# jdeschut/tunempc

Measured on AMD Instinct MI355X. Metric: stage-Hessian convexifications/sec at (nx+nu)=32, p=64, higher is better.
Workload: dtype f64

## Files before the change

### include/tunempc_hip.h

```cpp
#ifndef TUNEMPC_HIP_H
#define TUNEMPC_HIP_H

#include <stdint.h>

#ifdef __cplusplus
extern "C" {
#endif

#define TMPC_OK 0
#define TMPC_E_ARG (-1)
#define TMPC_E_UNSUPPORTED (-2)
#define TMPC_E_NOMEM (-3)
#define TMPC_E_HIP (-4)
#define TMPC_E_NODEVICE (-5)
#define TMPC_E_NOCONV (-6)

#define TMPC_STATUS_OPTIMAL 0
#define TMPC_STATUS_FEASIBLE 1
#define TMPC_STATUS_INFEASIBLE 2

#define TMPC_FLAG_NO_MFMA 1
#define TMPC_FLAG_PROFILE 2
#define TMPC_FLAG_FAST_EXIT 4

// ... 14 lines not shown
int tmpc_create_con(tmpc_handle** out, int chunk, int p, int nx, int mb, int ng, int nc);
int tmpc_destroy(tmpc_handle* h);
int tmpc_get_chunk(tmpc_handle* h);

int tmpc_set_options(tmpc_handle* h, double tol, double center_tol, int max_iter, int center_iter, int flags);

#define TMPC_TUNE_CHORD_STEP 1
#define TMPC_TUNE_SMALL_BLOCKS 2
#define TMPC_TUNE_EIG_PRETEST 3
#define TMPC_TUNE_FUSE_FWD 4
#define TMPC_TUNE_GRAPH 5
#define TMPC_TUNE_PERSISTENT 7
#define TMPC_TUNE_LOWP_SWITCH 8
#define TMPC_LOWP_SWITCH_DEFAULT 1e-5
#define TMPC_TUNE_LOWP_TRSM 9
int tmpc_set_tuning(tmpc_handle* h, int key, double value);
int tmpc_create_ex(tmpc_handle** out, int chunk, int p, int nx, int mb, int ng, int nc, int step3, int lanes);

int tmpc_set_tight(tmpc_handle* h, int enable, double tight_tol);

int tmpc_convexify_batch_host(tmpc_handle* h, int nb, const double* A, const double* B, const double* H,
                              double* Hc, double* dHc, double* P, double* alpha, double* beta, double* kappa,
                              int32_t* status, int32_t* iters, double* info);
int tmpc_convexify_batch_device(tmpc_handle* h, int nb, const double* dA, const double* dB, const double* dH,
                                double* dHc_out, double* ddHc_out, double* dP_out, double* d_alpha, double* d_beta,
                                double* d_kappa, int32_t* d_status, int32_t* d_iters, double* d_info, void* stream);

int tmpc_convexify_eq_batch_host(tmpc_handle* h, int nb, const double* A, const double* B, const double* H, const double* G,
                                 double* Hc, double* dHc, double* P, double* Fg, double* alpha, double* beta, double* kappa,
                                 int32_t* status, int32_t* iters, double* info);
// ... 77 lines not shown
```

### include/tunempc_hip_debug.h

```cpp
#ifndef TUNEMPC_HIP_DEBUG_H
#define TUNEMPC_HIP_DEBUG_H

#include "tunempc_hip.h"

#ifdef __cplusplus
extern "C" {
#endif

#define TMPC_DEBUG_FLAG_STOP_ASSEMBLED 8
#define TMPC_DEBUG_FLAG_NO_LIFT 16
#define TMPC_DEBUG_FLAG_NO_DMA 32
#define TMPC_DEBUG_FLAG_GENERIC_STAGE 64

int tmpc_debug_gemm_nt(tmpc_handle* h, double* C, const double* A, const double* B, int M, int N, int K, int mode, int lower);

int tmpc_debug_block_solve(tmpc_handle* h, int p, int d, const double* D, const double* Ccpl, const double* rhs, double* x, int32_t* nshift);

#define TMPC_DEBUG_FACTOR_PASS1 1
#define TMPC_DEBUG_FACTOR_FUSE_FWD1 2
#define TMPC_DEBUG_FACTOR_LOWP_TRSM 4
#define TMPC_DEBUG_FACTOR_DD 8
typedef struct {
  const double *D, *Ccpl, *Dlo, *Clo, *rhs;
  const int32_t *list, *lowp;
  double *oD, *oO, *oF, *oDdiag, *oX;
  float* oO32;
  double *oDl, *oOl, *oFl, *oXl;
  int32_t *nshift, *dims, *orient;
} tmpc_debug_factor_io;
int tmpc_debug_block_factor(tmpc_handle* h, int nb, int p, int d, int count, int mode, const tmpc_debug_factor_io* io);

int tmpc_debug_cr_schedule(int p, int32_t* out, int cap);

int tmpc_debug_get_multipliers(tmpc_handle* h, int nb, int nr, double* phi, double* z, double* dphi, double* dz);

int tmpc_debug_get_array(tmpc_handle* h, int which, uint64_t offset, uint64_t count, double* out);

int tmpc_debug_min_eig(tmpc_handle* h, int nmat, int n, const double* W, double* out);
int tmpc_debug_min_eig_lane(tmpc_handle* h, int nmat, int n, const double* W, double* out);

int tmpc_debug_factor_bench(tmpc_handle* h, int nb, int p, int d, int reps, double* ms_out2);

#ifdef __cplusplus
// ... 4 lines not shown
```

### tunempc_amd/_lib.py

```python
import ctypes as C
import os

import numpy as np

_HERE = os.path.dirname(os.path.abspath(__file__))
_LIB = None

INFO_STRIDE = 16
FLAG_NO_MFMA = 1
FLAG_PROFILE = 2
FLAG_FAST_EXIT = 4
STATUS_NAMES = {0: 'Optimal', 1: 'Feasible', 2: 'Infeasible'}

ARROW_LD = 32
EXPORTS = [
    'tmpc_device_count', 'tmpc_workspace_bytes', 'tmpc_workspace_bytes_eq', 'tmpc_workspace_bytes_con',
    'tmpc_create', 'tmpc_create_eq', 'tmpc_create_con', 'tmpc_destroy', 'tmpc_get_chunk', 'tmpc_set_options', 'tmpc_set_tight', 'tmpc_set_tuning', 'tmpc_create_ex',
    'tmpc_convexify_batch_host', 'tmpc_convexify_batch_device', 'tmpc_convexify_eq_batch_host', 'tmpc_convexify_step2_batch_host',
    'tmpc_convexify_con_batch_device', 'tmpc_workspace_bytes_step3', 'tmpc_create_step3', 'tmpc_convexify_step3_batch_host', 'tmpc_workspace_bytes_step3_con', 'tmpc_create_step3_con', 'tmpc_convexify_step3_con_batch_host', 'tmpc_convexify_step3_batch_device', 'tmpc_convexify_step3_con_batch_device', 'tmpc_supplement_batch_host', 'tmpc_supplement_terms_batch_host',
    'tmpc_tracking_reference_host', 'tmpc_eig_scan_host', 'tmpc_get_profile', 'tmpc_get_trace', 'tmpc_get_dual_host', 'tmpc_get_dual_con_host', 'tmpc_pack_sensitivities_host', 'tmpc_eig_clip_host',
    'tmpc_periodic_lqr_batch_host', 'tmpc_periodic_lqr_batch_device', 'tmpc_periodic_lqr_rows_batch_host', 'tmpc_periodic_lqr_rows_batch_device',
    'tmpc_periodic_lqr_ctg_batch_host', 'tmpc_periodic_lqr_ctg_batch_device',
    'tmpc_last_error', 'tmpc_version',
]
DEBUG_EXPORTS = [
    'tmpc_debug_gemm_nt', 'tmpc_debug_block_solve', 'tmpc_debug_cr_schedule', 'tmpc_debug_get_multipliers', 'tmpc_debug_get_array',
    'tmpc_debug_min_eig', 'tmpc_debug_min_eig_lane', 'tmpc_debug_factor_bench', 'tmpc_debug_block_factor',
]
FLAG_DEBUG_NO_DMA = 32
FACTOR_PASS1, FACTOR_FUSE_FWD1, FACTOR_LOWP_TRSM, FACTOR_DD = 1, 2, 4, 8


class _FactorIO(C.Structure):
    _fields_ = ([(n, C.POINTER(C.c_double)) for n in ('D', 'Ccpl', 'Dlo', 'Clo', 'rhs')] + [(n, C.POINTER(C.c_int32)) for n in ('list', 'lowp')] +
                [(n, C.POINTER(C.c_double)) for n in ('oD', 'oO', 'oF', 'oDdiag', 'oX')] + [('oO32', C.POINTER(C.c_float))] +
                [(n, C.POINTER(C.c_double)) for n in ('oDl', 'oOl', 'oFl', 'oXl')] + [(n, C.POINTER(C.c_int32)) for n in ('nshift', 'dims', 'orient')])


def library_path():
    return os.environ.get('TMPC_LIB') or os.path.join(_HERE, 'lib', 'libtunempc_hip.so')


def load_library():
    global _LIB
    if _LIB is not None:
        return _LIB
    path = library_path()
    if not os.path.exists(path):
        raise RuntimeError(
            f"tunempc_amd: HIP library not built ({path}); run `python -c 'import __graft_entry__ as g; g.build()'`"
            " -- there is no CPU fallback for the convexify hot path")
# ... 148 lines not shown
            _check(self.lib, self.lib.tmpc_create_step3_con(C.byref(self._h), int(chunk), self.p, self.nx, self.mb, self.ng, self.nc), 'tmpc_create_step3_con')
        elif self.step3:
            _check(self.lib, self.lib.tmpc_create_step3(C.byref(self._h), int(chunk), self.p, self.nx, self.mb), 'tmpc_create_step3')
        else:
            _check(self.lib, self.lib.tmpc_create_con(C.byref(self._h), int(chunk), self.p, self.nx, self.mb, self.ng, self.nc), 'tmpc_create_con')
        self.chunk = int(self.lib.tmpc_get_chunk(self._h))
        self.flags = int(flags)
        self.set_options(tol, center_tol, max_iter, center_iter, flags)

    def set_options(self, tol=None, center_tol=None, max_iter=None, center_iter=None, flags=None):
        if flags is not None:
            self.flags = int(flags)
        _check(self.lib, self.lib.tmpc_set_options(self._h, float(tol or 0.0), float(center_tol or 0.0),
                                                   int(max_iter or 0), int(center_iter or 0), self.flags), 'tmpc_set_options')

    def set_tuning(self, chord_step=None, small_blocks=None, eig_pretest=None, fuse_fwd=None, graph=None, persistent=None, lowp_switch=None, lowp_trsm=None):
        for key, v in ((1, chord_step), (2, small_blocks), (3, eig_pretest), (4, fuse_fwd), (5, graph), (7, persistent), (8, lowp_switch), (9, lowp_trsm)):
            if v is not None:
                _check(self.lib, self.lib.tmpc_set_tuning(self._h, key, float(v)), 'tmpc_set_tuning')

    def set_tight(self, enable=True, tight_tol=None):
        _check(self.lib, self.lib.tmpc_set_tight(self._h, 1 if enable else 0, float(tight_tol or 0.0)), 'tmpc_set_tight')

    def close(self):
        if getattr(self, '_h', None) is not None and self._h.value:
            self.lib.tmpc_destroy(self._h)
            self._h = C.c_void_p()

    def __del__(self):
        try:
            self.close()
        except Exception:
# ... 305 lines not shown
        nc = 3 if pass1 else 1
        if Ccpl.shape != D.shape or rhs.shape != ((nb, p, d, 3) if pass1 else (nb, p, d)):
            raise ValueError('debug_block_factor: D, Ccpl [nb, p, d, d] and rhs [nb, p, d] (pass 2) / [nb, p, d, 3] (pass 1) expected')
        plist = np.ascontiguousarray(np.arange(nb) if plist is None else plist, dtype=np.int32)
        lowp = None if lowp is None else np.ascontiguousarray(lowp, dtype=np.int32)
        if lowp is not None and lowp.shape != (nb,):
            raise ValueError('debug_block_factor: lowp [nb] expected')
        mode = (FACTOR_PASS1 if pass1 else 0) | (FACTOR_FUSE_FWD1 if fuse_fwd1 else 0) | (FACTOR_LOWP_TRSM if lowp_trsm else 0) | (FACTOR_DD if dd else 0)
        dp = (d + 15) // 16 * 16; ld32 = (dp + 31) // 32 * 32
        has32 = bool(lowp_trsm or (lowp is not None and lowp.any()))
        raw = dict(D=np.empty((nb, p, dp, dp)), O=np.empty((nb, p, dp, dp)), F=np.empty((nb, p, dp, dp)), Ddiag=np.empty((nb, p, dp)), X=np.empty((nb, p, dp, nc)),
                   O32=np.empty((nb, 2 * p, dp, ld32), np.float32) if has32 else None)
        if dd:
            raw.update(Dl=np.empty((nb, p, dp, dp)), Ol=np.empty((nb, p, dp, dp)), Fl=np.empty((nb, p, dp, dp)), Xl=np.empty((nb, p, dp, nc)))
        nshift = np.zeros(nb, np.int32); dims = np.zeros(4, np.int32); orient = np.zeros(p, np.int32)
        io = _FactorIO(D=_dptr(D), Ccpl=_dptr(Ccpl), Dlo=_dptr(Dlo), Clo=_dptr(Clo), rhs=_dptr(rhs), list=_iptr(plist), lowp=_iptr(lowp),
                       oD=_dptr(raw['D']), oO=_dptr(raw['O']), oF=_dptr(raw['F']), oDdiag=_dptr(raw['Ddiag']), oX=_dptr(raw['X']),
                       oO32=raw['O32'].ctypes.data_as(C.POINTER(C.c_float)) if has32 else None,
                       oDl=_dptr(raw.get('Dl')), oOl=_dptr(raw.get('Ol')), oFl=_dptr(raw.get('Fl')), oXl=_dptr(raw.get('Xl')),
                       nshift=_iptr(nshift), dims=_iptr(dims), orient=_iptr(orient))
        _check(self.lib, self.lib.tmpc_debug_block_factor(self._h, nb, p, d, len(plist), mode, C.byref(io)), 'tmpc_debug_block_factor')
        assert (int(dims[0]), int(dims[1]), int(dims[2]), bool(dims[3])) == (dp, ld32, nc, has32), dims
        raw.update(dp=dp, ld32=ld32)
        cut = lambda a: None if a is None else a[:, :, :d, :d].copy()
        vec = lambda a: None if a is None else (a[:, :, :d, :].copy() if pass1 else a[:, :, :d, 0].copy())
        out = dict(raw=raw, orient=orient, nshift=nshift, D=cut(raw['D']), L=np.tril(cut(raw['D'])), O=cut(raw['O']), F=cut(raw['F']), O32=cut(raw['O32']),
                   Ddiag=raw['Ddiag'][:, :, :d].copy(), x=vec(raw['X']))
        if dd:
            out.update(Dl=cut(raw['Dl']), Ll=np.tril(cut(raw['Dl'])), Ol=cut(raw['Ol']), Fl=cut(raw['Fl']), xl=vec(raw['Xl']))
        return out


def eig_clip(A, tol):
    lib = load_library()
    A = np.ascontiguousarray(A, dtype=np.float64)
    single = A.ndim == 2
    A3 = A[None] if single else A
    nb, n, n2 = A3.shape
    if n != n2:
        raise ValueError('square matrices expected')
    out = np.empty_like(A3); ev = np.empty((nb, n)); reg = np.empty(nb); sw = np.zeros(nb, dtype=np.int32)
    rc = lib.tmpc_eig_clip_host(nb, n, _dptr(A3), float(tol), _dptr(out), _dptr(ev), _dptr(reg), _iptr(sw))
# ... 124 lines not shown
```

### tunempc_amd/csrc/tmpc_api.hip

```cpp
#include <hip/hip_runtime.h>
#include <stdio.h>
#include <stdlib.h>
#include <new>
#include <string.h>
#include <algorithm>
#include <chrono>
#include <thread>
#include <mutex>
#include <condition_variable>
#include <functional>
#include <unistd.h>
#include <vector>

#include <string>
#include <unordered_map>

#include "../../include/tunempc_hip.h"
#include "../../include/tunempc_hip_debug.h"
#include "tmpc_common.h"
#include "tmpc_small.h"
#include "tmpc_stage.h"
#include "tmpc_schur.h"
#include "tmpc_factor.h"
#include "tmpc_cr.h"
// ... 92 lines not shown

struct tmpc_handle {
  Dims dm;
  int chunk;
  int nlanes;
  Opts opt;
  int flags;
  Lane lane[MAXL];
  void* slab;
  size_t slab_bytes;
  hipEvent_t ev_in;
  int device;
  CrSched sched;
  int* d_sched;
  int rs, mt;
  int tune_small, tune_pretest, tune_fuse, tune_graph, tune_persist, tune_lowp_trsm;
  void* dd_slab;
  size_t dd_bytes;
  int tight;
  double tight_tol;
};

static int cr_upload(const CrSched& sc, int** out) {
  std::vector<int> flat(sc.elim);
  flat.insert(flat.end(), sc.upd.begin(), sc.upd.end());
  flat.insert(flat.end(), sc.orient.begin(), sc.orient.end());
  *out = nullptr;
  if (hipMalloc(out, flat.size() * sizeof(int)) != hipSuccess) return TMPC_E_NOMEM;
  if (hipMemcpy(*out, flat.data(), flat.size() * sizeof(int), hipMemcpyHostToDevice) != hipSuccess) { hipFree(*out); *out = nullptr; return TMPC_E_HIP; }
  return TMPC_OK;
}
// ... 498 lines not shown
  } while (0)

static int run_chunk(tmpc_handle* h, Lane* ln, int nb, const double* dA, const double* dB, const double* dH, hipStream_t st,
                     const double* dG = nullptr, const int32_t* dncnt = nullptr, double rho = 0.0, bool step3 = false) {
  Dims dm = h->dm;
  dm.B = nb;
  if (!step3) dm.nT = 0;
  if (!dG) { dm.ng = 0; dm.nr = 0; dm.nz = 0; }
  dm.constr = (dG && dncnt && rho > 0.0) ? 1 : 0;
  if (dG && !dncnt) { dm.nr = dm.ng; dm.nz = dm.ng; }
  if (dG && dncnt && !dm.constr) dm.nz = dm.nr;
  const bool eq = dm.nr > 0;
  const bool t3 = dm.nT > 0;
  dm.dp = (dm.d + (eq ? dm.nz : 0) + (t3 ? dm.nT + 1 : 0) + 15) / 16 * 16;
  dm.nt = (dm.dp + TB - 1) / TB;
  dm.flags = (h->flags & TMPC_FLAG_NO_MFMA) | (h->tune_small ? 0 : DF_NO_SMALL) | ((h->flags & TMPC_DEBUG_FLAG_NO_DMA) ? DF_NO_DMA : 0);
  const size_t t3_lds = (size_t)(3 * (dm.nT + 1) + 8) * sizeof(double);
  const bool big = dm.n > NMAX || (h->flags & TMPC_DEBUG_FLAG_GENERIC_STAGE);
  const size_t t3_schur_lds = (size_t)((big ? 0 : 9 * 32 * T3_LD) + 2 * (dm.nT + 1)) * sizeof(double) + (size_t)(2 * (dm.nT + 1) + 2 * (dm.d + 1)) * sizeof(short) + 64;
  if (big && !ln->ws.bscr) {
    if (hipMalloc(&ln->big_scr, (size_t)h->dm.B * dm.p * BIG_SCR * dm.n * dm.n * sizeof(double)) != hipSuccess) { snprintf(g_err, sizeof(g_err), "hipMalloc of the generic-stage scratch failed"); return TMPC_E_NOMEM; }
    ln->ws.bscr = (double*)ln->big_scr;
  }
  WS wall = ln->ws;
  wall.A = dA; wall.Bm = dB; wall.H = dH; wall.G = dG; wall.ncnt = dncnt; wall.rho = rho;
  wall.cr_orient = h->d_sched + h->sched.elim.size() + h->sched.upd.size();
  WS w = wall;
  w.A = nullptr; w.Bm = nullptr; w.H = nullptr;
  int* alist = wall.alist;
  int* flist = wall.flist;
  wall.alist = nullptr;
// ... 348 lines not shown
  }
  tmpc_handle* h = new (std::nothrow) tmpc_handle();
  if (!h) return TMPC_E_NOMEM;
  h->slab = nullptr; h->d_sched = nullptr; h->ev_in = nullptr; h->dd_slab = nullptr; h->dd_bytes = 0; h->tight = 0; h->tight_tol = 0x1p-37;
  if (hipGetDevice(&h->device) != hipSuccess) { delete h; return TMPC_E_HIP; }
  int nl = (make_dims(1, p, nx, mb, ng, nc, step3).dp <= 64 && chunk >= 2) ? 2 : 1;
  if (lanes >= 1) nl = std::min(lanes, MAXL);
  nl = std::max(1, std::min(nl, chunk));
  h->nlanes = nl;
  const int cap = (chunk + nl - 1) / nl;
  h->chunk = cap * nl;
  h->dm = make_dims(cap, p, nx, mb, ng, nc, step3);
  h->sched = cr_build(p);
  h->rs = 0; h->mt = 0;
  h->tune_small = 1; h->tune_pretest = 1; h->tune_fuse = 1; h->tune_graph = 1; h->tune_persist = 1; h->tune_lowp_trsm = 1;
  h->opt.tol = 0x1p-25; h->opt.center_tol = 1e-9; h->opt.max_iter = 50; h->opt.center_iter = 12;
  h->opt.fast_exit = 0;
  h->opt.lowp_switch = TMPC_LOWP_SWITCH_DEFAULT;
  h->opt.chord_step = 10.0;
  h->flags = 0;
  WS tmp;
  const size_t lane_bytes = carve(tmp, h->dm, nullptr, nullptr);
  h->slab_bytes = lane_bytes * nl;
  if (hipMalloc(&h->slab, h->slab_bytes) != hipSuccess) {
    snprintf(g_err, sizeof(g_err), "hipMalloc(%zu bytes) failed", h->slab_bytes);
    delete h;
    return TMPC_E_NOMEM;
  }
  int rc = cr_upload(h->sched, &h->d_sched);
  bool ok = (rc == TMPC_OK) && hipEventCreateWithFlags(&h->ev_in, hipEventDisableTiming) == hipSuccess;
// ... 51 lines not shown
  return TMPC_OK;
}


int tmpc_set_tuning(tmpc_handle* h, int key, double value) {
  if (!h) return TMPC_E_ARG;
  switch (key) {
    case TMPC_TUNE_CHORD_STEP: if (!(value >= 0.0)) return TMPC_E_ARG; h->opt.chord_step = value; return TMPC_OK;
    case TMPC_TUNE_LOWP_SWITCH: if (!(value >= 0.0)) return TMPC_E_ARG; h->opt.lowp_switch = value; return TMPC_OK;
    case TMPC_TUNE_SMALL_BLOCKS: h->tune_small = value != 0.0; return TMPC_OK;
    case TMPC_TUNE_EIG_PRETEST: h->tune_pretest = value != 0.0; return TMPC_OK;
    case TMPC_TUNE_FUSE_FWD: h->tune_fuse = value != 0.0; return TMPC_OK;
    case TMPC_TUNE_GRAPH: h->tune_graph = value != 0.0; return TMPC_OK;
    case TMPC_TUNE_PERSISTENT: if (!(value >= 0.0 && value <= 2.0)) return TMPC_E_ARG; h->tune_persist = (int)value; return TMPC_OK;
    case TMPC_TUNE_LOWP_TRSM: h->tune_lowp_trsm = value != 0.0; return TMPC_OK;
    default: snprintf(g_err, sizeof(g_err), "tmpc_set_tuning: unknown key %d", key); return TMPC_E_ARG;
  }
}

int tmpc_set_tight(tmpc_handle* h, int enable, double tight_tol) {
  if (!h) return TMPC_E_ARG;
  if (!enable) { h->tight = 0; return TMPC_OK; }
  if (h->dm.nT > 0) { snprintf(g_err, sizeof(g_err), "tmpc_set_tight: Steps 1 and 2 only (no Step 3 handles)"); return TMPC_E_UNSUPPORTED; }
  if (h->dm.nr > 0 && (size_t)dd_aug_lds_doubles(h->dm.nr, h->dm.n, h->dm.nx) * sizeof(double) > 160 * 1024) {
    snprintf(g_err, sizeof(g_err), "tmpc_set_tight: %d rows per stage at nx = %d, nx + mb = %d: their double-double vectors do not fit the LDS (rows * (2 n + 2 nx) <= 4040)", h->dm.nr, h->dm.nx, h->dm.n);
    return TMPC_E_UNSUPPORTED;
  }
  if ((size_t)dd_solve_lds_doubles(h->dm.dp) * sizeof(double) > 160 * 1024) {
    snprintf(g_err, sizeof(g_err), "tmpc_set_tight: Schur blocks of %d do not fit the LDS image of the double-double substitution kernels (nx <= 51)", h->dm.dp);
    return TMPC_E_UNSUPPORTED;
// ... 810 lines not shown
        double dv = (i == j) ? 1.0 : 0.0, cv = 0.0;
        if (i < d && j < d) { dv = D[((size_t)k * d + i) * d + j]; cv = Ccpl[((size_t)k * d + i) * d + j]; }
        hD[k * bs + (size_t)i * dp + j] = dv;
        if (sc.orient[k]) hO[k * bs + (size_t)i * dp + j] = cv; else hO[k * bs + (size_t)j * dp + i] = cv;
      }
    for (int i = 0; i < d; ++i) hdd[(size_t)k * dp + i] = D[((size_t)k * d + i) * d + i];
  }
}

int tmpc_debug_block_solve(tmpc_handle* h, int p, int d, const double* D, const double* Ccpl, const double* rhs, double* x, int32_t* nshift) {
  if (!h || p < 1 || d < 1 || !D || !Ccpl || !rhs || !x) return TMPC_E_ARG;
  ON_DEVICE(h);
  CrBench cb;
  int rc = cb.init(1, p, d, h->flags, h->opt.lowp_switch >= 1.0);
  if (rc != TMPC_OK) return rc;
  const int dp = cb.dm.dp;
  const size_t bs = (size_t)dp * dp;
  std::vector<double> hD, hO, hdd, hz((size_t)p * dp, 0.0);
  cr_pack(cb.sc, p, d, dp, D, Ccpl, hD, hO, hdd);
  for (int k = 0; k < p; ++k) for (int i = 0; i < d; ++i) hz[(size_t)k * dp + i] = rhs[(size_t)k * d + i];
  HIPCHK(hipMemcpy(cb.w.D, hD.data(), p * bs * 8, hipMemcpyHostToDevice));
  HIPCHK(hipMemcpy(cb.w.O, hO.data(), p * bs * 8, hipMemcpyHostToDevice));
  HIPCHK(hipMemcpy(cb.w.Ddiag, hdd.data(), (size_t)p * dp * 8, hipMemcpyHostToDevice));
  HIPCHK(hipMemcpy(cb.w.Z, hz.data(), (size_t)p * dp * 8, hipMemcpyHostToDevice));
  cr_factor(cb.w, cb.dm, cb.sc, cb.d_sched, cb.w.alist, 1, 0, h->rs, h->mt, nullptr, nullptr, 0, cb.w.O32 ? 1 : 0);
  cr_solve(cb.w, cb.dm, cb.sc, cb.d_sched, cb.w.alist, 1, 0, 2);
  HIPCHK(hipDeviceSynchronize());
  HIPCHK(hipGetLastError());
  int hip_[IS];
  HIPCHK(hipMemcpy(hz.data(), cb.w.Z, (size_t)p * dp * 8, hipMemcpyDeviceToHost));
// ... 8 lines not shown
  if (mode & ~(TMPC_DEBUG_FACTOR_PASS1 | TMPC_DEBUG_FACTOR_FUSE_FWD1 | TMPC_DEBUG_FACTOR_LOWP_TRSM | TMPC_DEBUG_FACTOR_DD)) return TMPC_E_ARG;
  const bool pass1 = (mode & TMPC_DEBUG_FACTOR_PASS1) != 0, fuse = (mode & TMPC_DEBUG_FACTOR_FUSE_FWD1) != 0, ddm = (mode & TMPC_DEBUG_FACTOR_DD) != 0;
  std::vector<char> seen(nb, 0);
  int nlowp = 0, anylowp = 0;
  for (int i = 0; i < count; ++i) {
    const int b = io->list[i];
    if (b < 0 || b >= nb || seen[b]) { snprintf(g_err, sizeof(g_err), "tmpc_debug_block_factor: list entry %d is out of range or repeated", i); return TMPC_E_ARG; }
    seen[b] = 1;
    if (io->lowp && io->lowp[b]) ++nlowp;
  }
  for (int b = 0; b < nb && io->lowp; ++b) anylowp |= io->lowp[b] != 0;
  ON_DEVICE(h);
  CrBench cb;
  int rc = cb.init(nb, p, d, h->flags, false);
  if (rc != TMPC_OK) return rc;
  Dims& dm = cb.dm; WS& w = cb.w;
  if (h->flags & TMPC_DEBUG_FLAG_NO_DMA) dm.flags |= DF_NO_DMA;
  if (!h->tune_small) dm.flags |= DF_NO_SMALL;
  const int dp = dm.dp, ld32 = (dp + 31) & ~31, nc = pass1 ? 3 : 1;
  const size_t bs = (size_t)dp * dp, per = (size_t)p * bs, vl = (size_t)p * dp;
  if (solve_lds(dm) > 160 * 1024) return TMPC_E_UNSUPPORTED;
  const bool lowp_ok = !(dm.flags & (1 | DF_NO_DMA)) && dp > 64 && dm.nt <= TRR_NT;
  const bool fuse_ok = pass1 && !(dm.flags & (1 | DF_NO_DMA)) && p > 1 && dm.nt <= TRR_NT && !cr_small_levels(dm, cb.sc, nullptr);
  if ((anylowp || (mode & TMPC_DEBUG_FACTOR_LOWP_TRSM)) && (!lowp_ok || ddm)) { snprintf(g_err, sizeof(g_err), "tmpc_debug_block_factor: no float32 path at dp = %d with these flags", dp); return TMPC_E_ARG; }
  if (fuse && (!fuse_ok || ddm)) { snprintf(g_err, sizeof(g_err), "tmpc_debug_block_factor: no fused forward sweep at p = %d, dp = %d with these flags", p, dp); return TMPC_E_ARG; }
  DevBuf O32b, Dlb, Olb, Flb, Lilb, W3lb, Zlb;
  const size_t n32 = 2 * (size_t)nb * p * dp * ld32;
  if (anylowp || (mode & TMPC_DEBUG_FACTOR_LOWP_TRSM)) {
    if (O32b.alloc(n32 * sizeof(float)) != hipSuccess) return TMPC_E_NOMEM;
    HIPCHK(hipMemset(O32b.p, 0, n32 * sizeof(float)));
// ... 20 lines not shown
      std::fill(hz.begin(), hz.end(), 0.0);
      for (int k = 0; k < p; ++k) for (int i = 0; i < d; ++i) for (int q = 0; q < nc; ++q) hz[((size_t)k * dp + i) * nc + q] = io->rhs[(((size_t)b * p + k) * d + i) * nc + q];
      HIPCHK(hipMemcpy(w.D + b * per, hD.data(), per * 8, hipMemcpyHostToDevice));
      HIPCHK(hipMemcpy(w.O + b * per, hO.data(), per * 8, hipMemcpyHostToDevice));
      HIPCHK(hipMemcpy(w.Ddiag + b * vl, hdd.data(), vl * 8, hipMemcpyHostToDevice));
      HIPCHK(hipMemcpy(X + b * vl * nc, hz.data(), vl * nc * 8, hipMemcpyHostToDevice));
      if (ddm) {
        cr_pack(cb.sc, p, d, dp, io->Dlo ? io->Dlo + b * dd_ : zero.data(), io->Clo ? io->Clo + b * dd_ : zero.data(), hDl, hOl, hdl);
        for (int k = 0; k < p; ++k) for (int i = d; i < dp; ++i) hDl[k * bs + (size_t)i * dp + i] = 0.0;
        HIPCHK(hipMemcpy(w.Dl + b * per, hDl.data(), per * 8, hipMemcpyHostToDevice));
        HIPCHK(hipMemcpy(w.Ol + b * per, hOl.data(), per * 8, hipMemcpyHostToDevice));
      }
    }
  }
  if (count > 0) HIPCHK(hipMemcpy(w.alist, io->list, (size_t)count * sizeof(int), hipMemcpyHostToDevice));
  if (anylowp) {
    std::vector<int> hi((size_t)nb * IS, 0);
    for (int b = 0; b < nb; ++b) hi[(size_t)b * IS + I_LOWP] = io->lowp[b] ? 1 : 0;
    HIPCHK(hipMemcpy(w.iprob, hi.data(), hi.size() * sizeof(int), hipMemcpyHostToDevice));
  }
  if (count > 0) {
    const int pass = pass1 ? 1 : 2;
    if (ddm) {
      dd_factor(w, dm, cb.sc, cb.d_sched, w.alist, count, 0);
      rc = dd_solve(w, dm, cb.sc, cb.d_sched, w.alist, count, 0, pass, nb);
      if (rc != TMPC_OK) return rc;
    } else {
      cr_factor(w, dm, cb.sc, cb.d_sched, w.alist, count, 0, h->rs, h->mt, nullptr, nullptr, fuse ? 1 : 0, nlowp);
      cr_solve(w, dm, cb.sc, cb.d_sched, w.alist, count, 0, pass, fuse);
    }
// ... 7 lines not shown
  if (io->oX) HIPCHK(hipMemcpy(io->oX, X, nb * vl * nc * 8, hipMemcpyDeviceToHost));
  if (io->oO32 && w.O32) HIPCHK(hipMemcpy(io->oO32, w.O32, n32 * sizeof(float), hipMemcpyDeviceToHost));
  if (ddm) {
    if (io->oDl) HIPCHK(hipMemcpy(io->oDl, w.Dl, nb * per * 8, hipMemcpyDeviceToHost));
    if (io->oOl) HIPCHK(hipMemcpy(io->oOl, w.Ol, nb * per * 8, hipMemcpyDeviceToHost));
    if (io->oFl) HIPCHK(hipMemcpy(io->oFl, w.Fl, nb * per * 8, hipMemcpyDeviceToHost));
    if (io->oXl) HIPCHK(hipMemcpy(io->oXl, Xl, nb * vl * nc * 8, hipMemcpyDeviceToHost));
  }
  if (io->nshift) {
    std::vector<int> hi((size_t)nb * IS);
    HIPCHK(hipMemcpy(hi.data(), w.iprob, hi.size() * sizeof(int), hipMemcpyDeviceToHost));
    for (int b = 0; b < nb; ++b) io->nshift[b] = hi[(size_t)b * IS + I_NSHIFT];
  }
  if (io->dims) { io->dims[0] = dp; io->dims[1] = ld32; io->dims[2] = nc; io->dims[3] = w.O32 ? 1 : 0; }
  if (io->orient) for (int k = 0; k < p; ++k) io->orient[k] = cb.sc.orient[k];
  return TMPC_OK;
}

int tmpc_debug_factor_bench(tmpc_handle* h, int nb, int p, int d, int reps, double* ms_out2) {
  if (!h || nb < 1 || p < 1 || d < 1 || reps < 1 || !ms_out2) return TMPC_E_ARG;
  ON_DEVICE(h);
  CrBench cb;
  cb.ablate = (int)h->opt.lowp_switch - 2;
  int rc = cb.init(nb, p, d, h->flags, h->opt.lowp_switch >= 1.0);
  if (rc != TMPC_OK) return rc;
  const int dp = cb.dm.dp;
  const size_t bs = (size_t)dp * dp, per = (size_t)p * bs;
  std::vector<double> E((size_t)p * d * d), G((size_t)p * d * d), Dd((size_t)p * d * d, 0.0), Cc((size_t)p * d * d, 0.0);
  unsigned long long st = 88172645463325252ull;
  auto rnd = [&]() { st ^= st << 13; st ^= st >> 7; st ^= st << 17; return ((double)(st % 2000001) / 1000000.0 - 1.0) / sqrt((double)d); };
  for (auto& v : E) v = rnd();
  for (auto& v : G) v = rnd();
  for (int k = 0; k < p; ++k) {
    const int kn = (k + 1) % p;
    const double* Ek = &E[(size_t)k * d * d]; const double* Gk = &G[(size_t)k * d * d];
    for (int i = 0; i < d; ++i)
      for (int j = 0; j < d; ++j) {
        double ee = 0, gg = 0, eg = 0;
        for (int r = 0; r < d; ++r) { ee += Ek[r * d + i] * Ek[r * d + j]; gg += Gk[r * d + i] * Gk[r * d + j]; eg += Ek[r * d + i] * Gk[r * d + j]; }
        Dd[((size_t)k * d + i) * d + j] += ee + (i == j ? 1.0 : 0.0); Dd[((size_t)kn * d + i) * d + j] += gg;
// ... 47 lines not shown
```

### tunempc_amd/csrc/tmpc_common.h

```cpp
#pragma once
#include <hip/hip_runtime.h>
#include <stdint.h>

namespace tmpc {

#ifdef TMPC_CYCLE_PROF
__device__ unsigned long long g_prof[64];
__device__ int g_prof_cls;
#define TMPC_T(i) { if (blockIdx.x == 0 && threadIdx.x == 0) { const unsigned long long t_ = __builtin_readcyclecounter(); g_prof[(g_prof_cls & 7) * 8 + (i)] += t_ - tprev_; tprev_ = t_; } }
#define TMPC_T0() unsigned long long tprev_ = __builtin_readcyclecounter();
#define TMPC_TC(c, i) { if (blockIdx.x == 0 && threadIdx.x == 0) { const unsigned long long t_ = __builtin_readcyclecounter(); g_prof[(c) * 8 + (i)] += t_ - tprevc_; tprevc_ = t_; } }
#define TMPC_TC0() unsigned long long tprevc_ = __builtin_readcyclecounter();
#else
#define TMPC_TC(c, i)
#define TMPC_TC0()
#define TMPC_T(i)
#define TMPC_T0()
#endif



constexpr double ALPHA_MIN = 1e-8;
constexpr int TRACE_LEN = 80, TRACE_W = 10;
constexpr int TB = 64;
// ... 36 lines not shown
  int p;
  int nx, mb;
  int n;
  int d;
  int dp;
  int nt;
  int flags;
  int ng;
  int nr;
  int nz;
  int constr;
  int nT;
};
constexpr int DF_LOWP = 8;
constexpr int DF_LOWP_TRSM = 16;
constexpr int NGM = 31;
constexpr int NCM = 31;
constexpr int NRM = NGM + NCM, NZM = NRM + 2;
constexpr int NRS = 32, NZS = NRS + 2;
constexpr int NAM = 31;
constexpr int AEL = NAM + 1, AE = AEL * AEL;

struct Opts {
  double tol;
  double center_tol;
  int max_iter;
  int center_iter;
  double chord_step;
  int tight;
  double tight_tol;
// ... 80 lines not shown
```

### tunempc_amd/csrc/tmpc_cr.h

```cpp
#pragma once
#include <climits>
#include <vector>

#include "tmpc_common.h"
#include "tmpc_factor.h"
#include "tmpc_gemm_dma.h"

namespace tmpc {

constexpr int CR_EW = 8;
constexpr int CR_UW = 8;
enum { CE_NODE = 0, CE_NA, CE_NB, CE_EA, CE_EB, CE_FILL, CE_FX, CE_FACC };
enum { CU_NODE = 0, CU_E0, CU_S0, CU_E1, CU_S1 };

struct CrLevel { int eoff, nelim, uoff, nupd; };
struct CrSched {
  int p = 0;
  int prep = 0;
  std::vector<int> orient;
  std::vector<int> elim, upd;
  std::vector<CrLevel> lev;
};

static inline CrSched cr_build(int p) {
// ... 130 lines not shown

constexpr int UPD_DMA_DEPTH = 2;
template <bool USE_MFMA>
__global__ void __launch_bounds__(256, 2) k_cr_potrf(WS w, Dims dm, CrDev cr, int eoff, int nelim, int count) {
  const int it = cr_item(count * nelim);
  if (it < 0) return;
  extern __shared__ __attribute__((aligned(16))) double lds[];
  const int b = cr.alist[it / nelim];
  const int* er = cr.elim + (size_t)(eoff + it % nelim) * CR_EW;
  const int node = er[CE_NODE], dp = dm.dp;
  const size_t bs = (size_t)dp * dp;
  double* Dk = w.D + ((size_t)b * dm.p + node) * bs;
  double* Li = w.Linv + ((size_t)b * dm.p + node) * dm.nt * TB * TB;
  const double* dref = w.Ddiag + ((size_t)b * dm.p + node) * dp;
  double minr = 1.0;
  const int nbad = wg_block_column<USE_MFMA>(Dk, nullptr, nullptr, Li, dref, dp, lds, &minr);
  if (threadIdx.x == 0) {
    if (nbad) atomicAdd(w.iprob + (size_t)b * IS + I_NSHIFT, nbad);
    if (w.prob && minr < 1.0) atomic_min_pos(w.prob + (size_t)b * PS + P_MINPIV, minr);
  }
}

template <bool USE_MFMA, int NS>
__global__ void __launch_bounds__(256, 2) k_cr_trsm(WS w, Dims dm, CrDev cr, int eoff, int nelim, int count, int rs) {
  const int nstrip = (dm.dp + rs - 1) / rs;
  const int per = 2 * nstrip;
  const int it = cr_item(count * nelim * per);
  if (it < 0) return;
  extern __shared__ __attribute__((aligned(16))) double lds[];
  const int g = it / per, r = it - g * per;
  const int b = cr.alist[g / nelim];
// ... 586 lines not shown
  extern __shared__ __attribute__((aligned(16))) double lds[];
  const int b = cr.alist[it / nelim];
  const int* er = cr.elim + (size_t)(eoff + it % nelim) * CR_EW;
  const int node = er[CE_NODE], dp = dm.dp;
  double* Dk = w.D + ((size_t)b * dm.p + node) * (size_t)dp * dp;
  double* Li = w.Linv + ((size_t)b * dm.p + node) * dm.nt * TB * TB;
  const double* dref = w.Ddiag + ((size_t)b * dm.p + node) * dp;
  double* stat = lds + FACT_LDS_DOUBLES - 8;
  if (threadIdx.x == 0) { stat[0] = 0.0; stat[1] = 1.0; }
  for (int r = 0; r < dm.nt; ++r) {
    const int r0 = 64 * r, nb = (dp - r0 < 64) ? dp - r0 : 64;
    if (r > 0) {
      trd_strip<true>(Dk + (size_t)r0 * dp, Dk, Li, nb, r + 1, dp, it, lds);
      __syncthreads();
    }
    wg_potrf_inv(Dk + (size_t)r0 * dp + r0, dp, Li + (size_t)r * TB * TB, dref + r0, nb, lds, nullptr, stat, (it >> 5) & 3, r > 0);
  }
  if (threadIdx.x == 0) {
    const int nbad = (int)stat[0];
    const double minr = stat[1];
    if (nbad) atomicAdd(w.iprob + (size_t)b * IS + I_NSHIFT, nbad);
    if (w.prob && minr < 1.0) atomic_min_pos(w.prob + (size_t)b * PS + P_MINPIV, minr);
  }
}

template <bool USE_MFMA, int NS>
__global__ void __launch_bounds__(256, 2) k_cr_update(WS w, Dims dm, CrDev cr, int eoff, int nelim, int uoff, int nupd, int count, int mt) {
  const int nm = (dm.dp + mt - 1) / mt;
  const int ntl = nm * (nm + 1) / 2, ntf = nm * nm;
  const int per = nupd * ntl + nelim * ntf;
  const int it = cr_item(count * per);
// ... 233 lines not shown
```

### tunempc_amd/csrc/tmpc_factor.h

```cpp
#pragma once
#include "tmpc_common.h"

namespace tmpc {


#ifndef TMPC_LDP
#define TMPC_LDP 65
#endif
constexpr int FACT_LDS_DOUBLES = 2 * 64 * TMPC_LDP + 72 + 4 * 16 * 17 + 8;

enum { GM_SUB = 0, GM_SET = 1, GM_NEG = 2 };
constexpr int GM_NOTRI = -(1 << 30);

constexpr int SLD = 17, SUBD = 64 * SLD, SLABD = 2 * SUBD;
#ifdef TMPC_NT
#define TMPC_LD(p) __builtin_nontemporal_load(p)
#else
#define TMPC_LD(p) (*(p))
#endif
typedef const double __attribute__((address_space(1)))* gcptr;
typedef const double2_t __attribute__((address_space(1)))* gcptr2;
#define TMPC_LD4(dst, off, p, ok)                                                       \
  {                                                                                     \
    const double2_t u0_ = (ok) ? ((gcptr2)(p))[0] : (double2_t){0.0, 0.0};              \
// ... 275 lines not shown
  wave_lds_sync();
  double myrinv;
  {
    const double d = S[st.r * LDQ + st.r];
    double x = __builtin_amdgcn_rcp(d);
    x = fma(fma(-d, x, 1.0), x, x);
    x = fma(fma(-d, x, 1.0), x, x);
    myrinv = x;
  }
#pragma unroll
  for (int q = 0; q < 4; ++q) { const int c = 4 * q + st.g; Si[st.r * LDQ + c] = (c <= st.r) ? st.m[q] * myrinv : 0.0; }
  if (lane == 0) { stat[0] += st.nbad; stat[1] = fmin(stat[1], st.minr); }
  wave_lds_sync();
}

__device__ __noinline__ int wg_potrf_inv(double* T, int ldt, double* Ti, const double* dref, int nb, double* lds, double* minr, double* stat = nullptr, int sw = 0, bool preloaded = false) {
  const int tid = threadIdx.x, lane = tid & 63, wv = tid >> 6;
  TMPC_TC0()
  double* S = lds;
  double* Si = S + 64 * LDP;
  double* dr = Si + 64 * LDP;
  double* tmp = dr + 72 + wv * (16 * 17);
  {
    const int i = tid >> 2, j0 = (tid & 3) * 16;
    double2_t v[8];
    const bool on = i < nb && j0 < nb;
    if (on && !preloaded) {
      gcptr2 src = (gcptr2)(T + (size_t)i * ldt + j0);
#pragma unroll
      for (int q = 0; q < 8; ++q) v[q] = src[q];
#pragma unroll
      for (int q = 0; q < 8; ++q) { S[i * LDP + j0 + 2 * q] = v[q][0]; S[i * LDP + j0 + 2 * q + 1] = v[q][1]; }
    }
    if (on) {
#pragma unroll
      for (int q = 0; q < 8; ++q) { Si[i * LDP + j0 + 2 * q] = 0.0; Si[i * LDP + j0 + 2 * q + 1] = 0.0; }
    }
  }
  if (tid < nb) dr[tid] = dref[tid];
  if (tid == 0) { dr[65] = 0.0; dr[66] = 1.0; }
  __syncthreads();
  const int nbk = nb >> 4;
  TMPC_TC(7, 0)
  for (int jb = 0; jb < nbk; ++jb) {
    const int o = 16 * jb;
    if (wv == sw) wave_potrf16(S + o * LDP + o, Si + o * LDP + o, dr + o, dr + 65, lane);
    __syncthreads();
    TMPC_TC(7, 1)
    {
      const int bi = jb + 1 + wv;
      if (bi < nbk) {
        double4_t acc = (double4_t){0.0, 0.0, 0.0, 0.0};
        acc = mm16(S + 16 * bi * LDP + o, LDP, Si + o * LDP + o, 1, LDP, acc, 1.0, lane);
        store_d16(S + 16 * bi * LDP + o, LDP, acc, lane);
      }
    }
    __syncthreads();
    {
      int q = 0;
      for (int bi = jb + 1; bi < nbk; ++bi)
        for (int bj = jb + 1; bj <= bi; ++bj, ++q)
          if ((q & 3) == wv) {
            double* Cp = S + 16 * bi * LDP + 16 * bj;
            double4_t acc = load_d16(Cp, LDP, lane);
            acc = mm16(S + 16 * bi * LDP + o, LDP, S + 16 * bj * LDP + o, 1, LDP, acc, -1.0, lane);
            store_d16(Cp, LDP, acc, lane);
          }
    }
    __syncthreads();
    TMPC_TC(7, 2)
  }
  for (int bi = 1; bi < nbk; ++bi) {
    const int bj = wv;
    if (bj < bi) {
      double4_t acc = (double4_t){0.0, 0.0, 0.0, 0.0};
      for (int k = bj; k < bi; ++k) acc = mm16(S + 16 * bi * LDP + 16 * k, LDP, Si + 16 * k * LDP + 16 * bj, LDP, 1, acc, 1.0, lane);
      store_d16(tmp, 17, acc, lane);
      wave_lds_sync();
      double4_t r = (double4_t){0.0, 0.0, 0.0, 0.0};
      r = mm16(Si + 16 * bi * LDP + 16 * bi, LDP, tmp, 17, 1, r, -1.0, lane);
      store_d16(Si + 16 * bi * LDP + 16 * bj, LDP, r, lane);
    }
    __syncthreads();
  }
  TMPC_TC(7, 3)
  {
    const int i = tid >> 2, j0 = (tid & 3) * 16;
    if (i < nb && j0 < nb) {
      typedef double2_t __attribute__((address_space(1)))* gptr2;
      gptr2 dt = (gptr2)(T + (size_t)i * ldt + j0);
      gptr2 di = (gptr2)(Ti + i * TB + j0);
#pragma unroll
      for (int q = 0; q < 8; ++q) {
        const int j = j0 + 2 * q;
        di[q] = (double2_t){Si[i * LDP + j], Si[i * LDP + j + 1]};
        if (j + 1 <= i) dt[q] = (double2_t){S[i * LDP + j], S[i * LDP + j + 1]};
        else if (j <= i) T[(size_t)i * ldt + j] = S[i * LDP + j];
      }
    }
  }
  __syncthreads();
  TMPC_TC(7, 4)
  const int nb_bad = (int)dr[65];
  if (stat) { if (tid == 0) { stat[0] += dr[65]; stat[1] = fmin(stat[1], dr[66]); } }
  else *minr = fmin(*minr, dr[66]);
  __syncthreads();
  return nb_bad;
}

template <bool USE_MFMA>
__device__ __forceinline__ int wg_block_column(double* Dk, double* R1, double* R2, double* Linv_k, const double* dref,
                                               int dp, double* lds, double* minr) {
  int nbad = 0;
  int jt = 0;
  TMPC_TC0()
  for (int j0 = 0; j0 < dp; j0 += TB, ++jt) {
    const int nb = (dp - j0 < TB) ? dp - j0 : TB;
    if (j0 > 0) {
      wg_gemm_nt<USE_MFMA>(Dk + (size_t)j0 * dp + j0, dp, Dk + (size_t)j0 * dp, dp, Dk + (size_t)j0 * dp, dp, dp - j0, nb, j0, GM_SUB, false, lds);
      if (R1) wg_gemm_nt<USE_MFMA>(R1 + j0, dp, R1, dp, Dk + (size_t)j0 * dp, dp, dp, nb, j0, GM_SUB, false, lds);
      if (R2) wg_gemm_nt<USE_MFMA>(R2 + j0, dp, R2, dp, Dk + (size_t)j0 * dp, dp, dp, nb, j0, GM_SUB, false, lds);
    }
    TMPC_TC(6, 0)
    double* Ti = Linv_k + (size_t)jt * TB * TB;
    nbad += wg_potrf_inv(Dk + (size_t)j0 * dp + j0, dp, Ti, dref + j0, nb, lds, minr);
    TMPC_TC(6, 1)
    if (dp - j0 - nb > 0)
      wg_gemm_nt<USE_MFMA>(Dk + (size_t)(j0 + nb) * dp + j0, dp, Dk + (size_t)(j0 + nb) * dp + j0, dp, Ti, TB, dp - j0 - nb, nb, nb, GM_SET, false, lds);
    if (R1) wg_gemm_nt<USE_MFMA>(R1 + j0, dp, R1 + j0, dp, Ti, TB, dp, nb, nb, GM_SET, false, lds);
    if (R2) wg_gemm_nt<USE_MFMA>(R2 + j0, dp, R2 + j0, dp, Ti, TB, dp, nb, nb, GM_SET, false, lds);
    TMPC_TC(6, 2)
  }
  return nbad;
}

constexpr int NCP = 4;
constexpr int GKV = 16, GLDV = GKV + 1;

template <bool TRANS, bool LOWER = false, typename MT = double>
__device__ __forceinline__ void wg_gemv16(double* Y, int yld, const double* X, int xld, const MT* M, int ldm,
// ... 176 lines not shown
```

Before: 12080.

## Add lookahead scheduling to blocked Cholesky-inverse in wg_potrf_inv

Adds a lookahead mode to the 64x64 blocked Cholesky-and-inverse routine. While one wave factors the current 16x16 diagonal block, the other three waves apply the previous step's trailing updates and the inverse-row computations. The next panel and diagonal update are done right after, so the critical path no longer waits on the full trailing update each step. This also interleaves the separate inverse pass into the main loop and removes barriers, at the cost of more complex work assignment across waves. It is enabled by default through a new tuning flag and environment variable, and the debug interface now also returns Linv and the minimum pivot.

```diff
diff --git a/include/tunempc_hip.h b/include/tunempc_hip.h
--- a/include/tunempc_hip.h
+++ b/include/tunempc_hip.h
@@ -52,6 +52,7 @@
 #define TMPC_TUNE_LOWP_SWITCH 8
 #define TMPC_LOWP_SWITCH_DEFAULT 1e-5
 #define TMPC_TUNE_LOWP_TRSM 9
+#define TMPC_TUNE_POTRF_LOOKAHEAD 10
 int tmpc_set_tuning(tmpc_handle* h, int key, double value);
 int tmpc_create_ex(tmpc_handle** out, int chunk, int p, int nx, int mb, int ng, int nc, int step3, int lanes);
 
diff --git a/include/tunempc_hip_debug.h b/include/tunempc_hip_debug.h
--- a/include/tunempc_hip_debug.h
+++ b/include/tunempc_hip_debug.h
@@ -27,6 +27,7 @@
   float* oO32;
   double *oDl, *oOl, *oFl, *oXl;
   int32_t *nshift, *dims, *orient;
+  double *oLinv, *minpiv;
 } tmpc_debug_factor_io;
 int tmpc_debug_block_factor(tmpc_handle* h, int nb, int p, int d, int count, int mode, const tmpc_debug_factor_io* io);
 
diff --git a/tunempc_amd/_lib.py b/tunempc_amd/_lib.py
--- a/tunempc_amd/_lib.py
+++ b/tunempc_amd/_lib.py
@@ -34,7 +34,8 @@
 class _FactorIO(C.Structure):
     _fields_ = ([(n, C.POINTER(C.c_double)) for n in ('D', 'Ccpl', 'Dlo', 'Clo', 'rhs')] + [(n, C.POINTER(C.c_int32)) for n in ('list', 'lowp')] +
                 [(n, C.POINTER(C.c_double)) for n in ('oD', 'oO', 'oF', 'oDdiag', 'oX')] + [('oO32', C.POINTER(C.c_float))] +
-                [(n, C.POINTER(C.c_double)) for n in ('oDl', 'oOl', 'oFl', 'oXl')] + [(n, C.POINTER(C.c_int32)) for n in ('nshift', 'dims', 'orient')])
+                [(n, C.POINTER(C.c_double)) for n in ('oDl', 'oOl', 'oFl', 'oXl')] + [(n, C.POINTER(C.c_int32)) for n in ('nshift', 'dims', 'orient')] +
+                [(n, C.POINTER(C.c_double)) for n in ('oLinv', 'minpiv')])
 
 
 def library_path():
@@ -213,8 +214,8 @@
         _check(self.lib, self.lib.tmpc_set_options(self._h, float(tol or 0.0), float(center_tol or 0.0),
                                                    int(max_iter or 0), int(center_iter or 0), self.flags), 'tmpc_set_options')
 
-    def set_tuning(self, chord_step=None, small_blocks=None, eig_pretest=None, fuse_fwd=None, graph=None, persistent=None, lowp_switch=None, lowp_trsm=None):
-        for key, v in ((1, chord_step), (2, small_blocks), (3, eig_pretest), (4, fuse_fwd), (5, graph), (7, persistent), (8, lowp_switch), (9, lowp_trsm)):
+    def set_tuning(self, chord_step=None, small_blocks=None, eig_pretest=None, fuse_fwd=None, graph=None, persistent=None, lowp_switch=None, lowp_trsm=None, potrf_lookahead=None):
+        for key, v in ((1, chord_step), (2, small_blocks), (3, eig_pretest), (4, fuse_fwd), (5, graph), (7, persistent), (8, lowp_switch), (9, lowp_trsm), (10, potrf_lookahead)):
             if v is not None:
                 _check(self.lib, self.lib.tmpc_set_tuning(self._h, key, float(v)), 'tmpc_set_tuning')
 
@@ -550,18 +551,19 @@
         if dd:
             raw.update(Dl=np.empty((nb, p, dp, dp)), Ol=np.empty((nb, p, dp, dp)), Fl=np.empty((nb, p, dp, dp)), Xl=np.empty((nb, p, dp, nc)))
         nshift = np.zeros(nb, np.int32); dims = np.zeros(4, np.int32); orient = np.zeros(p, np.int32)
+        raw['Linv'] = np.empty((nb, p, (dp + 63) // 64, 64, 64)); minpiv = np.ones(nb)
         io = _FactorIO(D=_dptr(D), Ccpl=_dptr(Ccpl), Dlo=_dptr(Dlo), Clo=_dptr(Clo), rhs=_dptr(rhs), list=_iptr(plist), lowp=_iptr(lowp),
                        oD=_dptr(raw['D']), oO=_dptr(raw['O']), oF=_dptr(raw['F']), oDdiag=_dptr(raw['Ddiag']), oX=_dptr(raw['X']),
                        oO32=raw['O32'].ctypes.data_as(C.POINTER(C.c_float)) if has32 else None,
                        oDl=_dptr(raw.get('Dl')), oOl=_dptr(raw.get('Ol')), oFl=_dptr(raw.get('Fl')), oXl=_dptr(raw.get('Xl')),
-                       nshift=_iptr(nshift), dims=_iptr(dims), orient=_iptr(orient))
+                       nshift=_iptr(nshift), dims=_iptr(dims), orient=_iptr(orient), oLinv=_dptr(raw['Linv']), minpiv=_dptr(minpiv))
         _check(self.lib, self.lib.tmpc_debug_block_factor(self._h, nb, p, d, len(plist), mode, C.byref(io)), 'tmpc_debug_block_factor')
         assert (int(dims[0]), int(dims[1]), int(dims[2]), bool(dims[3])) == (dp, ld32, nc, has32), dims
         raw.update(dp=dp, ld32=ld32)
         cut = lambda a: None if a is None else a[:, :, :d, :d].copy()
         vec = lambda a: None if a is None else (a[:, :, :d, :].copy() if pass1 else a[:, :, :d, 0].copy())
         out = dict(raw=raw, orient=orient, nshift=nshift, D=cut(raw['D']), L=np.tril(cut(raw['D'])), O=cut(raw['O']), F=cut(raw['F']), O32=cut(raw['O32']),
-                   Ddiag=raw['Ddiag'][:, :, :d].copy(), x=vec(raw['X']))
+                   Ddiag=raw['Ddiag'][:, :, :d].copy(), x=vec(raw['X']), Linv=raw['Linv'], minpiv=minpiv)
         if dd:
             out.update(Dl=cut(raw['Dl']), Ll=np.tril(cut(raw['Dl'])), Ol=cut(raw['Ol']), Fl=cut(raw['Fl']), xl=vec(raw['Xl']))
         return out
diff --git a/tunempc_amd/csrc/tmpc_api.hip b/tunempc_amd/csrc/tmpc_api.hip
--- a/tunempc_amd/csrc/tmpc_api.hip
+++ b/tunempc_amd/csrc/tmpc_api.hip
@@ -130,7 +130,7 @@
   CrSched sched;
   int* d_sched;
   int rs, mt;
-  int tune_small, tune_pretest, tune_fuse, tune_graph, tune_persist, tune_lowp_trsm;
+  int tune_small, tune_pretest, tune_fuse, tune_graph, tune_persist, tune_lowp_trsm, tune_potrf_la;
   void* dd_slab;
   size_t dd_bytes;
   int tight;
@@ -659,7 +659,7 @@
   const bool t3 = dm.nT > 0;
   dm.dp = (dm.d + (eq ? dm.nz : 0) + (t3 ? dm.nT + 1 : 0) + 15) / 16 * 16;
   dm.nt = (dm.dp + TB - 1) / TB;
-  dm.flags = (h->flags & TMPC_FLAG_NO_MFMA) | (h->tune_small ? 0 : DF_NO_SMALL) | ((h->flags & TMPC_DEBUG_FLAG_NO_DMA) ? DF_NO_DMA : 0);
+  dm.flags = (h->flags & TMPC_FLAG_NO_MFMA) | (h->tune_small ? 0 : DF_NO_SMALL) | ((h->flags & TMPC_DEBUG_FLAG_NO_DMA) ? DF_NO_DMA : 0) | (h->tune_potrf_la ? DF_POTRF_LA : 0);
   const size_t t3_lds = (size_t)(3 * (dm.nT + 1) + 8) * sizeof(double);
   const bool big = dm.n > NMAX || (h->flags & TMPC_DEBUG_FLAG_GENERIC_STAGE);
   const size_t t3_schur_lds = (size_t)((big ? 0 : 9 * 32 * T3_LD) + 2 * (dm.nT + 1)) * sizeof(double) + (size_t)(2 * (dm.nT + 1) + 2 * (dm.d + 1)) * sizeof(short) + 64;
@@ -1038,6 +1038,8 @@
   h->sched = cr_build(p);
   h->rs = 0; h->mt = 0;
   h->tune_small = 1; h->tune_pretest = 1; h->tune_fuse = 1; h->tune_graph = 1; h->tune_persist = 1; h->tune_lowp_trsm = 1;
+  h->tune_potrf_la = 1;
+  if (const char* e = getenv("TMPC_POTRF_LOOKAHEAD")) h->tune_potrf_la = atoi(e) != 0;
   h->opt.tol = 0x1p-25; h->opt.center_tol = 1e-9; h->opt.max_iter = 50; h->opt.center_iter = 12;
   h->opt.fast_exit = 0;
   h->opt.lowp_switch = TMPC_LOWP_SWITCH_DEFAULT;
@@ -1119,6 +1121,7 @@
     case TMPC_TUNE_GRAPH: h->tune_graph = value != 0.0; return TMPC_OK;
     case TMPC_TUNE_PERSISTENT: if (!(value >= 0.0 && value <= 2.0)) return TMPC_E_ARG; h->tune_persist = (int)value; return TMPC_OK;
     case TMPC_TUNE_LOWP_TRSM: h->tune_lowp_trsm = value != 0.0; return TMPC_OK;
+    case TMPC_TUNE_POTRF_LOOKAHEAD: h->tune_potrf_la = value != 0.0; return TMPC_OK;
     default: snprintf(g_err, sizeof(g_err), "tmpc_set_tuning: unknown key %d", key); return TMPC_E_ARG;
   }
 }
@@ -1959,6 +1962,7 @@
   CrBench cb;
   int rc = cb.init(1, p, d, h->flags, h->opt.lowp_switch >= 1.0);
   if (rc != TMPC_OK) return rc;
+  if (h->tune_potrf_la) cb.dm.flags |= DF_POTRF_LA;
   const int dp = cb.dm.dp;
   const size_t bs = (size_t)dp * dp;
   std::vector<double> hD, hO, hdd, hz((size_t)p * dp, 0.0);
@@ -1997,6 +2001,7 @@
   CrBench cb;
   int rc = cb.init(nb, p, d, h->flags, false);
   if (rc != TMPC_OK) return rc;
+  if (h->tune_potrf_la) cb.dm.flags |= DF_POTRF_LA;
   Dims& dm = cb.dm; WS& w = cb.w;
   if (h->flags & TMPC_DEBUG_FLAG_NO_DMA) dm.flags |= DF_NO_DMA;
   if (!h->tune_small) dm.flags |= DF_NO_SMALL;
@@ -2047,6 +2052,7 @@
     }
   }
   if (count > 0) HIPCHK(hipMemcpy(w.alist, io->list, (size_t)count * sizeof(int), hipMemcpyHostToDevice));
+  if (io->oLinv) HIPCHK(hipMemset(w.Linv, 0, (size_t)nb * p * dm.nt * TB * TB * 8));
   if (anylowp) {
     std::vector<int> hi((size_t)nb * IS, 0);
     for (int b = 0; b < nb; ++b) hi[(size_t)b * IS + I_LOWP] = io->lowp[b] ? 1 : 0;
@@ -2084,6 +2090,12 @@
   }
   if (io->dims) { io->dims[0] = dp; io->dims[1] = ld32; io->dims[2] = nc; io->dims[3] = w.O32 ? 1 : 0; }
   if (io->orient) for (int k = 0; k < p; ++k) io->orient[k] = cb.sc.orient[k];
+  if (io->oLinv) HIPCHK(hipMemcpy(io->oLinv, w.Linv, (size_t)nb * p * dm.nt * TB * TB * 8, hipMemcpyDeviceToHost));
+  if (io->minpiv) {
+    std::vector<double> hp((size_t)nb * PS);
+    HIPCHK(hipMemcpy(hp.data(), w.prob, hp.size() * 8, hipMemcpyDeviceToHost));
+    for (int b = 0; b < nb; ++b) io->minpiv[b] = hp[(size_t)b * PS + P_MINPIV];
+  }
   return TMPC_OK;
 }
 
@@ -2094,6 +2106,7 @@
   cb.ablate = (int)h->opt.lowp_switch - 2;
   int rc = cb.init(nb, p, d, h->flags, h->opt.lowp_switch >= 1.0);
   if (rc != TMPC_OK) return rc;
+  if (h->tune_potrf_la) cb.dm.flags |= DF_POTRF_LA;
   const int dp = cb.dm.dp;
   const size_t bs = (size_t)dp * dp, per = (size_t)p * bs;
   std::vector<double> E((size_t)p * d * d), G((size_t)p * d * d), Dd((size_t)p * d * d, 0.0), Cc((size_t)p * d * d, 0.0);
diff --git a/tunempc_amd/csrc/tmpc_common.h b/tunempc_amd/csrc/tmpc_common.h
--- a/tunempc_amd/csrc/tmpc_common.h
+++ b/tunempc_amd/csrc/tmpc_common.h
@@ -74,6 +74,7 @@
 };
 constexpr int DF_LOWP = 8;
 constexpr int DF_LOWP_TRSM = 16;
+constexpr int DF_POTRF_LA = 32;
 constexpr int NGM = 31;
 constexpr int NCM = 31;
 constexpr int NRM = NGM + NCM, NZM = NRM + 2;
diff --git a/tunempc_amd/csrc/tmpc_cr.h b/tunempc_amd/csrc/tmpc_cr.h
--- a/tunempc_amd/csrc/tmpc_cr.h
+++ b/tunempc_amd/csrc/tmpc_cr.h
@@ -168,7 +168,7 @@
   double* Li = w.Linv + ((size_t)b * dm.p + node) * dm.nt * TB * TB;
   const double* dref = w.Ddiag + ((size_t)b * dm.p + node) * dp;
   double minr = 1.0;
-  const int nbad = wg_block_column<USE_MFMA>(Dk, nullptr, nullptr, Li, dref, dp, lds, &minr);
+  const int nbad = wg_block_column<USE_MFMA>(Dk, nullptr, nullptr, Li, dref, dp, lds, &minr, (dm.flags & DF_POTRF_LA) != 0);
   if (threadIdx.x == 0) {
     if (nbad) atomicAdd(w.iprob + (size_t)b * IS + I_NSHIFT, nbad);
     if (w.prob && minr < 1.0) atomic_min_pos(w.prob + (size_t)b * PS + P_MINPIV, minr);
@@ -785,7 +785,7 @@
       trd_strip<true>(Dk + (size_t)r0 * dp, Dk, Li, nb, r + 1, dp, it, lds);
       __syncthreads();
     }
-    wg_potrf_inv(Dk + (size_t)r0 * dp + r0, dp, Li + (size_t)r * TB * TB, dref + r0, nb, lds, nullptr, stat, (it >> 5) & 3, r > 0);
+    wg_potrf_inv(Dk + (size_t)r0 * dp + r0, dp, Li + (size_t)r * TB * TB, dref + r0, nb, lds, nullptr, stat, (it >> 5) & 3, r > 0, (dm.flags & DF_POTRF_LA) != 0);
   }
   if (threadIdx.x == 0) {
     const int nbad = (int)stat[0];
diff --git a/tunempc_amd/csrc/tmpc_factor.h b/tunempc_amd/csrc/tmpc_factor.h
--- a/tunempc_amd/csrc/tmpc_factor.h
+++ b/tunempc_amd/csrc/tmpc_factor.h
@@ -313,7 +313,7 @@
   wave_lds_sync();
 }
 
-__device__ __noinline__ int wg_potrf_inv(double* T, int ldt, double* Ti, const double* dref, int nb, double* lds, double* minr, double* stat = nullptr, int sw = 0, bool preloaded = false) {
+__device__ __noinline__ int wg_potrf_inv(double* T, int ldt, double* Ti, const double* dref, int nb, double* lds, double* minr, double* stat = nullptr, int sw = 0, bool preloaded = false, bool la = false) {
   const int tid = threadIdx.x, lane = tid & 63, wv = tid >> 6;
   TMPC_TC0()
   double* S = lds;
@@ -341,46 +341,76 @@
   __syncthreads();
   const int nbk = nb >> 4;
   TMPC_TC(7, 0)
+  auto panel = [&](int bi, int o) {
+    double4_t acc = (double4_t){0.0, 0.0, 0.0, 0.0};
+    acc = mm16(S + 16 * bi * LDP + o, LDP, Si + o * LDP + o, 1, LDP, acc, 1.0, lane);
+    store_d16(S + 16 * bi * LDP + o, LDP, acc, lane);
+  };
+  auto trail = [&](int bi, int bj, int o) {
+    double* Cp = S + 16 * bi * LDP + 16 * bj;
+    double4_t acc = load_d16(Cp, LDP, lane);
+    acc = mm16(S + 16 * bi * LDP + o, LDP, S + 16 * bj * LDP + o, 1, LDP, acc, -1.0, lane);
+    store_d16(Cp, LDP, acc, lane);
+  };
+  auto inv_sum = [&](int bi, int bj) {
+    double4_t acc = (double4_t){0.0, 0.0, 0.0, 0.0};
+    for (int k = bj; k < bi; ++k) acc = mm16(S + 16 * bi * LDP + 16 * k, LDP, Si + 16 * k * LDP + 16 * bj, LDP, 1, acc, 1.0, lane);
+    store_d16(tmp, 17, acc, lane);
+    wave_lds_sync();
+  };
+  auto inv_fin = [&](int bi, int bj) {
+    double4_t r = (double4_t){0.0, 0.0, 0.0, 0.0};
+    r = mm16(Si + 16 * bi * LDP + 16 * bi, LDP, tmp, 17, 1, r, -1.0, lane);
+    store_d16(Si + 16 * bi * LDP + 16 * bj, LDP, r, lane);
+  };
+  const int hw = (wv - sw - 1) & 3;
   for (int jb = 0; jb < nbk; ++jb) {
     const int o = 16 * jb;
     if (wv == sw) wave_potrf16(S + o * LDP + o, Si + o * LDP + o, dr + o, dr + 65, lane);
+    else if (la && jb > 0) {
+      if (jb + 1 < nbk) {
+        int q = 0;
+        for (int bi = jb + 1; bi < nbk; ++bi)
+          for (int bj = jb; bj <= bi; ++bj, ++q)
+            if (q % 3 == hw) trail(bi, bj, o - 16);
+        for (int bj = 0; bj + 1 < jb; ++bj, ++q)
+          if (q % 3 == hw) { inv_sum(jb - 1, bj); inv_fin(jb - 1, bj); wave_lds_sync(); }
+      } else {
+        if (hw + 1 < jb) { inv_sum(jb - 1, hw); inv_fin(jb - 1, hw); wave_lds_sync(); }
+        if (hw < jb) inv_sum(jb, hw);
+      }
+    }
     __syncthreads();
+    if (la) {
+      TMPC_TC(7, 5)
+      if (jb + 1 < nbk) {
+        if (wv == sw) { panel(jb + 1, o); wave_lds_sync(); trail(jb + 1, jb + 1, o); }
+        else if (jb + 2 + hw < nbk) panel(jb + 2 + hw, o);
+        __syncthreads();
+      }
+      TMPC_TC(7, 6)
+      continue;
+    }
     TMPC_TC(7, 1)
-    {
-      const int bi = jb + 1 + wv;
-      if (bi < nbk) {
-        double4_t acc = (double4_t){0.0, 0.0, 0.0, 0.0};
-        acc = mm16(S + 16 * bi * LDP + o, LDP, Si + o * LDP + o, 1, LDP, acc, 1.0, lane);
-        store_d16(S + 16 * bi * LDP + o, LDP, acc, lane);
-      }
-    }
+    if (jb + 1 + wv < nbk) panel(jb + 1 + wv, o);
     __syncthreads();
     {
       int q = 0;
       for (int bi = jb + 1; bi < nbk; ++bi)
         for (int bj = jb + 1; bj <= bi; ++bj, ++q)
-          if ((q & 3) == wv) {
-            double* Cp = S + 16 * bi * LDP + 16 * bj;
-            double4_t acc = load_d16(Cp, LDP, lane);
-            acc = mm16(S + 16 * bi * LDP + o, LDP, S + 16 * bj * LDP + o, 1, LDP, acc, -1.0, lane);
-            store_d16(Cp, LDP, acc, lane);
-          }
+          if ((q & 3) == wv) trail(bi, bj, o);
     }
     __syncthreads();
     TMPC_TC(7, 2)
   }
-  for (int bi = 1; bi < nbk; ++bi) {
-    const int bj = wv;
-    if (bj < bi) {
-      double4_t acc = (double4_t){0.0, 0.0, 0.0, 0.0};
-      for (int k = bj; k < bi; ++k) acc = mm16(S + 16 * bi * LDP + 16 * k, LDP, Si + 16 * k * LDP + 16 * bj, LDP, 1, acc, 1.0, lane);
-      store_d16(tmp, 17, acc, lane);
-      wave_lds_sync();
-      double4_t r = (double4_t){0.0, 0.0, 0.0, 0.0};
-      r = mm16(Si + 16 * bi * LDP + 16 * bi, LDP, tmp, 17, 1, r, -1.0, lane);
-      store_d16(Si + 16 * bi * LDP + 16 * bj, LDP, r, lane);
-    }
+  if (la) {
+    if (hw < nbk - 1) inv_fin(nbk - 1, hw);
     __syncthreads();
+  } else {
+    for (int bi = 1; bi < nbk; ++bi) {
+      if (wv < bi) { inv_sum(bi, wv); inv_fin(bi, wv); }
+      __syncthreads();
+    }
   }
   TMPC_TC(7, 3)
   {
@@ -409,7 +439,7 @@
 
 template <bool USE_MFMA>
 __device__ __forceinline__ int wg_block_column(double* Dk, double* R1, double* R2, double* Linv_k, const double* dref,
-                                               int dp, double* lds, double* minr) {
+                                               int dp, double* lds, double* minr, bool la = false) {
   int nbad = 0;
   int jt = 0;
   TMPC_TC0()
@@ -422,7 +452,7 @@
     }
     TMPC_TC(6, 0)
     double* Ti = Linv_k + (size_t)jt * TB * TB;
-    nbad += wg_potrf_inv(Dk + (size_t)j0 * dp + j0, dp, Ti, dref + j0, nb, lds, minr);
+    nbad += wg_potrf_inv(Dk + (size_t)j0 * dp + j0, dp, Ti, dref + j0, nb, lds, minr, nullptr, 0, false, la);
     TMPC_TC(6, 1)
     if (dp - j0 - nb > 0)
       wg_gemm_nt<USE_MFMA>(Dk + (size_t)(j0 + nb) * dp + j0, dp, Dk + (size_t)(j0 + nb) * dp + j0, dp, Ti, TB, dp - j0 - nb, nb, nb, GM_SET, false, lds);
```

Result: no change. 12130, median of 6 (+0.4%).
